# althonos/pyopal

Hardware: AMD Instinct MI355X
Metric: GCUPS (billion DP cells/s) SW score-only, 53aa query vs 1Mx300aa DB (higher is better)
Workload: dtype u16; 1 GPU; sw_score q53 (README.md:86) vs 1000000x300 uniform-random proteins per GPU, BLOSUM62, gap_open 3, gap_extend 1; value: blocking miopalSearch, scores in the caller's pinned host array (value_device_results: scores left in HBM); targets_per_gpu=1000000, target_length=300, query_length=53

## Files before the change

### pyopal_amd/csrc/common.h

```cpp
#pragma once
#include <hip/hip_runtime.h>
#include <stdint.h>
#include "launch_layer.h"

namespace miopal {

constexpr int kLanes = 64;
constexpr int kGroupTargets = 128;
constexpr int kMaxAlphabet = 32;
constexpr int kMaxStripRows = 64;

enum Region : int { kLastCell = 0, kLastRow = 1, kLastRowCol = 2, kAllCells = 3 };
struct DpRules {
    int topGap;
    int leftGap;
    int floor0;
    int region;
};

struct InterseqArgs {
    const uint2* pack;
    const int64_t* groupOff;
    const int* groupChunks;
    int nGroups;
// ... 17 lines not shown
    int* unitFlags;
    uint2* unitPartial;
    int scoreBias;
    int biasedLimit;
    int biasedZero;
    int capGroups, capChunks;
    int tailThrottle;
    unsigned long long* stripKeys;
    int* stripAbort;
    int stripAbortAt;
    int* stripGaveUp;
    int batchGroups;
    const int32_t* known;
    int32_t* directOut;
    int32_t* directEndI;
    int32_t* directEndJ;
    const int32_t* directIds;
    int directN;
    int splitMode;
    int splitBlocks;
    const int64_t* chunkPrefix;
    uint4* splitState;
    int* splitFlags;
    int stripSpinCap;
    int faultUnit1;
    unsigned long long* stripTiming;
    uint2* boundary[2];
    const int64_t* boundaryOff;
};

struct BatchArgs {
    const uint2* pack;
    const int64_t* groupOff;
    const int* groupChunks;
    const int32_t* lens;
    const int32_t* ids;
    int nPacked;
    int64_t sliceStart;
    const int16_t* profiles;
    int nSymbols;
    const int* qLens;
    const int* qRows;
    int nQueries;
    int unitsPerQuery;
    const int* unitFirst;
    int* unitCounter;
// ... 163 lines not shown
    kSwShifted = 6
};
constexpr int kSwShiftZero = 0x1000;
constexpr int kUnsignedDiagZero = 0x1000;
hipError_t launchInterseq(const InterseqArgs& a, int rowsPerStrip, int waves, InterseqFlavour flavour,
                          bool locate, hipStream_t stream);
__host__ __device__ constexpr int pairRowSlots(int rowsPerStrip) { return ((rowsPerStrip + 3) / 4) | 1; }
__host__ __device__ constexpr size_t pairLdsBytes(int rowsPerStrip, int nSymbols) {
    return (size_t)nSymbols * nSymbols * pairRowSlots(rowsPerStrip) * 16;
}
bool interseqPairFits(int rowsPerStrip, int nSymbols);
enum PairFlavour : int {
    kPairSwInt16 = 0,
    kPairSwHalf = 1,
    kPairSwBiased = 2,
    kPairGlobalBiased = 3,
    kPairSwStrips = 4,
    kPairGlobalStrips = 5
};
constexpr int kPairStripsFirst = 32;
constexpr int kPairStripsMaxRows = 52, kPairStripsMaxRowsLoc = 48;
constexpr int kPairStripsMaxRowsKnown = 40;
constexpr int kPairWavesPerGroup = 12;
inline size_t splitStateBytes(int rows) { return (size_t)((2 * rows + 1 + 3) / 4) * kLanes * 16; }
constexpr int kBiasedScoreLimit = 25600;
constexpr int kBiasedMaxMagnitude = 1024;
constexpr int kBiasedMaxExt = 512;
constexpr int kBiasedMaxStepUp = 0x1000;
constexpr int kBiasedPad = -1024;
constexpr int kLocZeroPattern = 0x0C00;
constexpr int kLocGuardBand = 0x0800;
constexpr int kLocMaxShift = 4096;
inline int locRowBitsHost(int rows) { return rows <= 16 ? 4 : rows <= 32 ? 5 : 6; }
hipError_t launchInterseqPair(const InterseqArgs& a, int rowsPerStrip, PairFlavour flavour, int computeUnits,
                              hipStream_t stream, bool locate = false);
struct ArithSwI16;
struct ArithSwF16;
struct ArithI16;
struct ArithI16Diag;
struct ArithU16Diag;
struct ArithSwU16;
constexpr int kPairUnitCounts = 8, kPairUnitSpan = 2 * kPairUnitCounts;
template <typename Arith, bool TRACK_ALL, bool LOC>
hipError_t launchFlavour(const InterseqArgs& a, int rowsPerStrip, int waves, hipStream_t stream);
template <typename Arith>
hipError_t launchPairFlavour(const InterseqArgs& a, int rowsPerStrip, int computeUnits, hipStream_t stream);
// ... 81 lines not shown
```

### pyopal_amd/csrc/host.hip

```cpp
#include <algorithm>
#include <atomic>
#include <chrono>
#include <condition_variable>
#if defined(__x86_64__)
#include <immintrin.h>
#endif
#include <cstdarg>
#include <cstdio>
#include <cstdlib>
#include <cstring>
#include <deque>
#include <functional>
#include <exception>
#include <ctime>
#include <list>
#include <map>
#include <memory>
#include <mutex>
#include <new>
#include <numeric>
#include <string>
#include <sys/mman.h>
#include <thread>
#include <vector>
// ... 527 lines not shown
    for (int k = 0; k < 4; ++k) counts[k] = g_lastRouting[k];
}

int miopalLastFullRouting(void) { return g_lastFullRouting; }

void miopalLastBatchRouting(int64_t counts[4]) {
    if (!counts) return;
    for (int k = 0; k < 4; ++k) counts[k] = g_lastBatchRouting[k];
}

int miopalLastKernelTime(MiopalDb* db, float* ms) {
    if (!db || !ms) return 0;
    std::lock_guard<std::mutex> g(db->timingMutex);
    *ms = 0.f;
    Workspace* ws = db->lastTimed;
    if (!ws) return 0;
    int n = 0;
    for (auto& ev : ws->timings) {
        float t = 0.f;
        if (hipEventSynchronize(ev.second) == hipSuccess &&
            hipEventElapsedTime(&t, ev.first, ev.second) == hipSuccess) {
            *ms += t;
            ++n;
        }
        (void)hipEventDestroy(ev.first);
        (void)hipEventDestroy(ev.second);
    }
    ws->timings.clear();
    return n;
}

int miopalSearchDeviceScores(MiopalDb* db, const unsigned char* query, int queryLength, int gapOpen,
                             int gapExt, const int* scoreMatrix, int alphabetLength, int mode,
                             int64_t start, int64_t end, int* deviceScores, void* stream) {
    return guarded([&]() -> int {
    RC_TRY(validate(db, query, queryLength, scoreMatrix, alphabetLength, OPAL_SEARCH_SCORE, mode, start, end));
    if (end == start) return 0;
    if (!deviceScores) return fail(MIOPAL_ERR_BAD_ARGUMENT, "null device score buffer");
    HIP_TRY(hipSetDevice(db->device));
    WorkspaceLease lease(db);
    RC_TRY(lease.acquireExternal((hipStream_t)stream));
    Search s{db, lease.ws, (hipStream_t)stream, query, queryLength, gapOpen, gapExt, alphabetLength,
             OPAL_SEARCH_SCORE, mode, scoreMatrix, start, end, end - start};
    RC_TRY(s.prepare());
    RC_TRY(s.scorePass((int32_t*)deviceScores, nullptr, nullptr));
    if (s.d_stripError) {
// ... 473 lines not shown
```

### pyopal_amd/csrc/host_search.inc

```
static inline int reservedCus(const MiopalDb* db) {
    const int opt = db->optReserveCus.load(std::memory_order_relaxed);
    if (opt >= 0) return opt;
    if (const char* r = tuned(Tune::RESERVE_CUS)) return std::max(0, atoi(r));
    return -1;
}
static inline bool smallSearchAllowed(const MiopalDb* db) {
    const int opt = db->optSmallSearch.load(std::memory_order_relaxed);
    if (opt >= 0) return opt != 0;
    return !tuned(Tune::NO_SMALL_SEARCH);
}

struct Search {
    MiopalDb* db;
    Workspace* ws;
    hipStream_t stream;
    const unsigned char* query;
    int Q, open, ext, A, searchType, mode;
    const int* matrix;
    int64_t start, end;
    int64_t n;
    const int* pssmRows = nullptr;
    int at(int i, int t) const { return pssmRows ? pssmRows[(size_t)i * A + t] : matrix[query[i] * A + t]; }
    int maxScore = 0, minScore = 0;
    int64_t balancedChunks = 0;
// ... 781 lines not shown
            ia.directN = view->nPacked;
            ia.overflow = nullptr;
            directScatter = true;
        }
        const PairFlavour pf = p.globalPair ? kPairGlobalBiased : p.biased ? kPairSwBiased : p.halfFloat ? kPairSwHalf : kPairSwInt16;
        size_t splitFlags = 0;
        if (pf == kPairSwBiased && !p.locate) {
            const char* cs = tuned(Tune::COLUMN_SPLIT);
            const bool recompute = cs && !strcmp(cs, "recompute");
            const int forced = cs && !recompute ? std::max(0, atoi(cs)) : 0;
            int64_t chunks = view->totalChunks;
            for (int g = 0; g < p.firstGroup; ++g) chunks -= view->groupChunksHost[g];
            const int blocks = (int)std::min<int64_t>(forced > 0 ? std::min(forced, pairUnits) : std::max(1, std::min(pairUnits, ia.nGroups)),
                                                      chunks / kPairWavesPerGroup);
            const int64_t wavefronts = (int64_t)blocks * kPairWavesPerGroup;
            if (blocks >= 1 && (recompute || forced > 0 || (!cs && uniform && chunks / wavefronts >= longest))) {
                void* st;
                RC_TRY(ws->get(kSplitState, (size_t)(wavefronts + 1) * splitStateBytes(p.pairRows), &st));
                ia.splitMode = recompute ? 2 : 1;
                ia.splitBlocks = blocks;
                ia.chunkPrefix = view->d_chunkPrefix;
                ia.splitState = (uint4*)st;
                splitFlags = (size_t)wavefronts + 1;
            }
        }
        RC_TRY(ws->get(kWorkCounter, (1 + splitFlags) * sizeof(int), &wc));
        HIP_TRY(hipMemsetAsync(wc, 0, (1 + splitFlags) * sizeof(int), stream));
        ia.workCounter = (int*)wc;
        if (splitFlags) ia.splitFlags = (int*)wc + 1;
        unsigned long long* simdFinish = nullptr;
        const int finishSlots = 1 + 4 * pairUnits;
        if (pf == kPairSwBiased && tuned(Tune::STRIP_TIMING)) {
            void* tb;
            RC_TRY(ws->get(kStripTiming, finishSlots * sizeof(unsigned long long), &tb));
            HIP_TRY(hipMemsetAsync(tb, 0, finishSlots * sizeof(unsigned long long), stream));
            HIP_TRY(hipMemsetAsync(tb, 0xff, sizeof(unsigned long long), stream));
            ia.stripTiming = simdFinish = (unsigned long long*)tb;
        }
        g_lastRouting[1] = 2 + (int)pf + (ia.splitMode ? 64 : 0);
        const hipError_t pe = tuned(Tune::TEST_REFUSE_PAIR_LAUNCH)
                                  ? hipErrorInvalidValue
                                  : launchInterseqPair(ia, (p.biased || p.globalPair) ? p.pairRows : p.rows, pf, pairUnits, stream, p.locate);
        if (pe == hipSuccess && simdFinish) {
            std::vector<unsigned long long> t((size_t)finishSlots);
            HIP_TRY(hipMemcpyAsync(t.data(), simdFinish, t.size() * sizeof(unsigned long long), hipMemcpyDeviceToHost, stream));
            HIP_TRY(hipStreamSynchronize(stream));
            double sum = 0, last = 0, first = 1e30;
            int n = 0;
            for (int i = 1; i < finishSlots; ++i) {
                if (t[i] == 0) continue;
                const double us = (double)(t[i] - t[0]) / 100.0;
                sum += us;
                last = std::max(last, us);
                first = std::min(first, us);
                ++n;
            }
            if (n > 0)
                fprintf(stderr, "[miopal] headline timing (%d SIMDs, %d groups, %d rows): finish mean %.1f us  first %.1f  last %.1f  "
                                "last - mean %.1f us\n",
                        n, ia.nGroups, p.pairRows, sum / n, first, last, last - sum / n);
        }
        done->directScatter = directScatter;
        done->launch = pe;
        return 0;
    }

    int scatterResults(const View* view, const ScorePlan& p, const InterseqArgs& ia, const PassBuffers& b, bool sideEmpty, bool forked,
                       bool directScatter, int32_t* d_score, int32_t* d_endI, int32_t* d_endJ) {
        const int nScatter = view->nPacked - p.packedSkip;
        if (p.keyed) {
            if (p.firstPos != 0 || !sideEmpty || forked)
                return fail(MIOPAL_ERR_INTERNAL, "segmented view with side jobs");
            HIP_TRY(launchScatterKeyed(ia.score, ia.endI, ia.endJ, (const uint8_t*)b.vo, view->d_ids,
                                       view->d_segStart, nScatter, start, (unsigned long long*)b.keys,
                                       p.mayOverflow ? (int32_t*)b.ct : nullptr, stream, p.keyBias));
            HIP_TRY(launchDecodeKeys((const unsigned long long*)b.keys, (int)n, d_score, d_endI, d_endJ, stream, p.keyBias));
        } else if (!directScatter) {
            HIP_TRY(launchScatter(ia.score + p.packedSkip, (const uint8_t*)b.vo + p.packedSkip, view->d_ids + p.packedSkip,
                                  nScatter, start, d_score, p.mayOverflow ? (int32_t*)b.ct : nullptr, p.overlap > 0,
                                  stream));
            if (p.locate)
                HIP_TRY(launchScatterEnds(ia.endI + p.packedSkip, ia.endJ + p.packedSkip, view->d_ids + p.packedSkip,
                                          nScatter, start, d_endI, d_endJ, stream));
// ... 33 lines not shown
        if (p.keyed) {
            RC_TRY(ws->get(kKeys, (size_t)n * sizeof(unsigned long long), &b.keys));
            HIP_TRY(hipMemsetAsync(b.keys, 0, (size_t)n * sizeof(unsigned long long), stream));
        } else if (p.overlap > 0) {
            if (p.keyBias) HIP_TRY(launchFillInt32(d_score, (int)n, INT32_MIN, stream));
            else HIP_TRY(hipMemsetAsync(d_score, 0, (size_t)n * sizeof(int32_t), stream));
        }
        planGeneralStrips(view.get(), p);
        planSwPairStrips(view.get(), useHalf, p);
        planGlobalPairStrips(view.get(), useHalf, p);
        planSideCut(view.get(), p, sideJobs);

        if (view->nGroups > p.firstGroup) {
            planLanes(view.get(), useHalf, p, jobs, sideJobs);
            const std::vector<int16_t> prof = buildProfile(p);
            bool forked = sideForked;
            bool directScatter = false;
            RC_TRY(forkSideJobs(p, sideJobs, d_score, d_endI, d_endJ, &forked, spt));
            InterseqArgs ia{};
            RC_TRY(prepareLaunch(view.get(), p, prof, b, ia));
            const bool timed = db->profiling.load() != 0;
            EventPair ev;
            if (timed) {
                HIP_TRY(hipEventCreate(&ev.e0));
                HIP_TRY(hipEventCreate(&ev.e1));
                HIP_TRY(hipEventRecord(ev.e0, stream));
            }
            g_lastRouting[1] = 1 + 32 * (int)p.flavour;
            if (p.pairStrips) {
                StripsLaunch sl;
                RC_TRY(prepareStripsLaunch(p, ia, &sl));
                hipError_t pe = hipSuccess;
                if (p.probeEnds) {
                    StripsProbe probe;
                    RC_TRY(probeStripsEnds(p, ia, sl, &probe));
                    pe = probe.launch;
                    if (pe == hipSuccess && 2 * probe.beyond >= probe.lanes) {
                        stripsEndsDeclined = true;
                        twoPassEnds = !tuned(Tune::NO_TWO_PASS_ENDS);
                        return scorePassImpl(d_score, d_endI, d_endJ, useHalf);
                    }
                }
                if (pe == hipSuccess) RC_TRY(launchStripsSweeps(view.get(), p, ia, sl, &pe));
                if (pe != hipSuccess) {
                    (void)hipGetLastError();
                    (p.globalStrips ? globalStripsRefused : pairStripsRefused) = true;
                    if (tuned(Tune::VERBOSE))
                        fprintf(stderr, "miopal: multi-strip pair-table kernel refused (%s), using the general kernel\n",
// ... 72 lines not shown
```

### pyopal_amd/csrc/host_types.inc

```
struct View {
    int64_t start = 0, end = 0;
    int overlap = 0;
    int stride = 0;
    int32_t* d_segStart = nullptr;
    int nPacked = 0;
    int nGroups = 0;
    int maxPackedLen = 0;
    std::vector<int> groupChunksHost;
    int64_t totalChunks = 0;
    std::vector<int32_t> ids;
    std::vector<int32_t> longIds;
    int32_t* d_ids = nullptr;
    int32_t* d_lens = nullptr;
    uint2* d_pack = nullptr;
    int64_t* d_groupOff = nullptr;
    int* d_groupChunks = nullptr;
    int64_t* d_boundaryOff = nullptr;
    int64_t* d_chunkPrefix = nullptr;
    size_t deviceBytes = 0;
    void* d_meta = nullptr;
    bool packPending = false;
    PackArgs pendingPack{};
    size_t packCap = 0, metaCap = 0;
    ~View() {
        if (d_pack) (void)hipFree(d_pack);
        if (d_meta) (void)hipFree(d_meta);
    }
};

}

struct MiopalDb {
    int device = 0;
    int ordinal = 0;
    std::atomic<int> optReserveCus{-1};
    std::atomic<int> optSmallSearch{-1};
    int alphabet = 0;
    int64_t count = 0;
    int64_t total = 0;
    int64_t maxLen = 0;
    int computeUnits = 256;
    std::vector<int64_t> offsets;
    uint8_t* d_residues = nullptr;
    int64_t* d_offsets = nullptr;
    size_t residueCap = 0, offsetsCap = 0;
    std::vector<std::pair<void*, size_t>> spareBlocks;

    struct ViewSlot {
        int64_t start, end;
// ... 133 lines not shown
```

### pyopal_amd/csrc/host_workspace.inc

```
enum Slot {
    kQuery, kMatrix, kProfile, kViewScore, kViewOvf, kCounter, kBoundary0, kBoundary1,
    kScore, kEndI, kEndJ, kJobs, kPairB0, kPairB1, kAuxJobs, kAuxPairB0, kAuxPairB1, kRScore, kRI, kRJ, kDirs, kOps, kOpsOff,
    kOpsLen, kOvfHost, kWorkCounter, kViewEndI, kViewEndJ, kStartQ, kStartT, kMismatch, kCompactOps, kTraceScore, kOpsTotals, kSortBins, kSortedJobs, kScanOrder, kKeys, kHeadWaves, kHeadDirs, kUnitState, kUnitPartial, kStripKeys,
    kPairStripState, kPairStripPartial, kPairStripSpare, kAuxPairStripState, kAuxPairStripPartial, kPairStripError, kStripTiming,
    kBatchProfiles, kBatchMeta, kBatchOverflow,
    kPairListQ, kPairListT, kPairListTOff, kPairListQBase, kPairListQOff, kPairListBoundary,
    kTopScratch,
    kPssmRows,
    kSplitState,
    kSlots
};

namespace unpack {
#if defined(__x86_64__)
__attribute__((target("bmi2"))) inline void pieces(uint8_t* dst, const uint8_t* packed, int64_t n8) {
    for (int64_t k = 0; k < n8; ++k) {
        uint16_t w;
        memcpy(&w, packed + 2 * k, 2);
        const uint64_t v = __builtin_ia32_pdep_di((uint64_t)w, 0x0303030303030303ull);
        memcpy(dst + 8 * k, &v, 8);
    }
}
inline bool havePdep() {
    static const bool yes = __builtin_cpu_supports("bmi2");
    return yes;
}
__attribute__((target("avx512f,avx512bw,avx512vbmi"))) inline void pieces64(uint8_t* dst, const uint8_t* packed, int64_t n64,
                                                                              bool stream) {
    const __m512i from = _mm512_set1_epi64((long long)0x0e0c0a0806040200ull);
    const __m512i low2 = _mm512_set1_epi8(3);
    if (stream) {
        for (int64_t k = 0; k < n64; ++k) {
// ... 202 lines not shown
inline bool haveAvx512() { return false; }
#endif
inline void copyLarge(void* dst, const void* src, size_t bytes) {
    if (bytes < (256u << 10) || !haveAvx512()) {
        memcpy(dst, src, bytes);
        return;
    }
    uint8_t* d = (uint8_t*)dst;
    const uint8_t* s = (const uint8_t*)src;
    const size_t lead = (64 - (reinterpret_cast<uintptr_t>(d) & 63)) & 63;
    memcpy(d, s, lead);
    const size_t lines = (bytes - lead) / 64;
    streamLines(d + lead, s + lead, lines);
    memcpy(d + lead + 64 * lines, s + lead + 64 * lines, bytes - lead - 64 * lines);
}
}

struct Workspace {
    hipStream_t stream = nullptr;
    bool ownsStream = false;
    void* buf[kSlots] = {};
    size_t cap[kSlots] = {};
    uint64_t usedBy[kSlots] = {};
    uint64_t leaseStamp = 0;
    std::mutex busy;
    std::vector<std::pair<hipEvent_t, hipEvent_t>> timings;
    hipStream_t aux = nullptr;
    hipEvent_t evFork = nullptr, evJoin = nullptr;

    void* pinned = nullptr;
    size_t pinnedCap = 0, pinnedUsed = 0;
    uint64_t stagingGeneration = 0;
    struct Pending { void* dst; size_t off, bytes; bool onAux = false; };
    std::vector<Pending> pending;
    std::vector<int32_t> hostScratchA, hostScratchB;

    static void copyOut(void* dst, const char* src, size_t bytes) {
        constexpr size_t kPiece = 4u << 20;
        if (bytes < 2 * kPiece) {
            unpack::copyLarge(dst, src, bytes);
            return;
        }
        const int nThreads = (int)std::min<size_t>(4, bytes / kPiece);
        const size_t share = ((bytes / nThreads) + 4095) & ~(size_t)4095;
        std::vector<std::thread> pool;
        for (int t = 1; t < nThreads; ++t) {
            const size_t lo = share * t, hi = std::min(bytes, lo + share);
            if (lo >= hi) continue;
            try {
// ... 120 lines not shown
            (void)hipGetLastError();
            least = greatest = 0;
        }
        if (greatest != least) HIP_TRY(hipStreamCreateWithPriority(&aux, hipStreamNonBlocking, greatest));
        else HIP_TRY(hipStreamCreateWithFlags(&aux, hipStreamNonBlocking));
        HIP_TRY(hipEventCreateWithFlags(&evFork, hipEventDisableTiming));
        HIP_TRY(hipEventCreateWithFlags(&evJoin, hipEventDisableTiming));
        return 0;
    }

    int get(int slot, size_t bytes, void** out) {
        if (bytes == 0) bytes = 16;
        usedBy[slot] = leaseStamp;
        if (cap[slot] < bytes) {
            if (buf[slot]) {
                HIP_TRY(hipStreamSynchronize(stream));
                HIP_TRY(hipFree(buf[slot]));
                buf[slot] = nullptr;
                cap[slot] = 0;
            }
            size_t want = bytes + bytes / 8 + 256;
            HIP_TRY(hipMalloc(&buf[slot], want));
            cap[slot] = want;
            if (want > (512u << 20) && tuned(Tune::VERBOSE))
                fprintf(stderr, "miopal: workspace slot %d grows to %zu MiB\n", slot, want >> 20);
        }
        *out = buf[slot];
        return 0;
    }
    bool tryGet(int slot, size_t bytes, void** out) {
        usedBy[slot] = leaseStamp;
        if (cap[slot] >= bytes) {
            *out = buf[slot];
            return true;
        }
        if (buf[slot]) {
            (void)hipStreamSynchronize(stream);
            (void)hipFree(buf[slot]);
            buf[slot] = nullptr;
            cap[slot] = 0;
        }
        if (hipMalloc(&buf[slot], bytes) != hipSuccess) {
            (void)hipGetLastError();
            buf[slot] = nullptr;
            return false;
        }
        cap[slot] = bytes;
        if (bytes > (512u << 20) && tuned(Tune::VERBOSE))
            fprintf(stderr, "miopal: workspace slot %d grows to %zu MiB\n", slot, bytes >> 20);
        *out = buf[slot];
        return true;
    }
    size_t bytes() const {
        size_t t = 0;
        for (size_t c : cap) t += c;
        return t;
    }
    size_t trimTo(size_t keep, bool staleOnly = false) {
        size_t freed = 0;
        for (int pass = 0; pass < (staleOnly ? 1 : 2); ++pass)
        while (bytes() > keep) {
            int big = -1;
            for (int k = 0; k < kSlots; ++k)
                if (buf[k] && (pass == 1 || usedBy[k] != leaseStamp) && (big < 0 || cap[k] > cap[big])) big = k;
            if (big < 0) break;
            (void)hipFree(buf[big]);
            freed += cap[big];
            buf[big] = nullptr;
            cap[big] = 0;
        }
        return freed;
    }
    ~Workspace() {
        for (auto& ev : timings) {
            (void)hipEventDestroy(ev.first);
            (void)hipEventDestroy(ev.second);
        }
        for (void* p : buf)
            if (p) (void)hipFree(p);
        if (pinned) (void)hipHostFree(pinned);
        if (evFork) (void)hipEventDestroy(evFork);
        if (evJoin) (void)hipEventDestroy(evJoin);
        if (aux) (void)hipStreamDestroy(aux);
        if (ownsStream && stream) (void)hipStreamDestroy(stream);
    }
};
```

### pyopal_amd/csrc/interseq_impl.h

```cpp
#pragma once
#include <algorithm>

#include <type_traits>

#include "common.h"

namespace miopal {

typedef short s16x2 __attribute__((ext_vector_type(2)));
typedef unsigned short u16x2 __attribute__((ext_vector_type(2)));
typedef _Float16 f16x2 __attribute__((ext_vector_type(2)));

static __device__ __forceinline__ uint32_t pk_add_sat_i16(uint32_t a, uint32_t b) {
    s16x2 r = __builtin_elementwise_add_sat(__builtin_bit_cast(s16x2, a), __builtin_bit_cast(s16x2, b));
    return __builtin_bit_cast(uint32_t, r);
}
static __device__ __forceinline__ uint32_t pk_sub_sat_i16(uint32_t a, uint32_t b) {
    s16x2 r = __builtin_elementwise_sub_sat(__builtin_bit_cast(s16x2, a), __builtin_bit_cast(s16x2, b));
    return __builtin_bit_cast(uint32_t, r);
}
static __device__ __forceinline__ uint32_t pk_max_i16(uint32_t a, uint32_t b) {
    s16x2 r = __builtin_elementwise_max(__builtin_bit_cast(s16x2, a), __builtin_bit_cast(s16x2, b));
    return __builtin_bit_cast(uint32_t, r);
}
// ... 905 lines not shown
    __device__ __forceinline__ void begin(int lane) const {
        if (MIOPAL_STRIP_PACE && lane == 0) *mine = 0;
    }
    __device__ __forceinline__ void end(int lane) const {
        if (MIOPAL_STRIP_PACE && lane == 0) *mine = INT32_MAX;
    }
    __device__ __forceinline__ void step(int c, int lane, bool fixed) const {
        if (!MIOPAL_STRIP_PACE || fixed) return;
        if (lane == 0) *mine = c;
        const int4 p = *simdRow;
        const int behind = __builtin_amdgcn_readfirstlane(min(min(p.x, p.y), min(p.z, p.w)));
        if (c <= behind) __builtin_amdgcn_s_setprio(2);
        else __builtin_amdgcn_s_setprio(0);
    }
};

#ifndef MIOPAL_HEADLINE_PACE
#define MIOPAL_HEADLINE_PACE 1
#endif
#ifndef MIOPAL_HEADLINE_TIMING
#define MIOPAL_HEADLINE_TIMING 0
#endif

struct SplitState {
    __amdgpu_buffer_rsrc_t rsrc;
    __device__ __forceinline__ explicit SplitState(void* base)
        : rsrc(__builtin_amdgcn_make_buffer_rsrc(base, 0, 0x7ffffff0, 0x00020000)) {}
    static __device__ __forceinline__ int at(int quad) {
        int offset = quad * (kLanes * 16);
        asm volatile("" : "+s"(offset));
        return offset;
    }
    __device__ __forceinline__ StripU4 load(int quad, int lane) const {
        return __builtin_amdgcn_raw_buffer_load_b128(rsrc, lane * 16, at(quad), 16 );
    }
    __device__ __forceinline__ void store(int quad, int lane, StripU4 v) const {
        __builtin_amdgcn_raw_buffer_store_b128(v, rsrc, lane * 16, at(quad), 16 );
    }
};
constexpr int kSplitPolls = 256;
__host__ __device__ constexpr int splitStateQuads(int rows) { return (2 * rows + 1 + 3) / 4; }

template <int R, bool LOC, bool SPLIT = false>
__global__ __launch_bounds__(kPairWaves * kLanes) void interseq_pair_biased_kernel(InterseqArgs a) {
    static_assert(!(SPLIT && LOC), "the column split carries no end locations");
    constexpr int SLOTS = PairLayout<R>::kRowSlots;
    constexpr int NB4 = (R + 3) / 4;
    constexpr int kBits = LOC ? locRowBits(R) : 0;
    constexpr int kRowMask = (1 << kBits) - 1;
    extern __shared__ uint4 pairs[];
#if MIOPAL_HEADLINE_TIMING
    const unsigned long long born = __builtin_amdgcn_s_memrealtime();
#endif

    const int lane = threadIdx.x & 63;
    const int nSym = a.nSymbols;
    const int ext = a.gapExt << kBits;
    const uint32_t ext2 = both(ext), openMinusExt2 = both((a.gapOpen << kBits) - ext);
    const uint32_t zero2 = both(LOC ? kLocZero : kBiasedZero);

    {
        const int16_t* gp = a.profile;
        uint32_t* pw = reinterpret_cast<uint32_t*>(pairs);
        const int total = nSym * nSym * R;
        for (int idx = threadIdx.x; idx < total; idx += kPairWaves * kLanes) {
            const int row = idx / R, r = idx - row * R;
            const int tA = row / nSym, tB = row - tA * nSym;
            constexpr int kPadPattern = LOC ? -kLocGuard : kBiasedPadScore;
            const int vA = gp[tA * a.qPad + r], vB = gp[tB * a.qPad + r];
            const int sA = (vA == kBiasedPadScore ? kPadPattern : vA << kBits) + ext;
            const int sB = (vB == kBiasedPadScore ? kPadPattern : vB << kBits) + ext;
            pw[row * (SLOTS * 4) + r] = (uint32_t)(sB * 65536 + sA);
        }
    }
    int* simdTaken = reinterpret_cast<int*>(pairs + nSym * nSym * SLOTS);
    if (threadIdx.x < 4) simdTaken[threadIdx.x] = 0;
    __syncthreads();
    SimdPace pace;
    if (MIOPAL_HEADLINE_PACE) pace.init(simdTaken + 4, lane);

    const int wave = __builtin_amdgcn_readfirstlane((int)(threadIdx.x >> 6));
    constexpr int kTier[4][3] = {{0, 6, 11}, {1, 7, 8}, {2, 5, 9}, {3, 4, 10}};
    const int tier = kTier[wave & 3][wave >> 2];
    const int firstDynamic = kPairWaves * gridDim.x;
    const int simd = (int)__builtin_amdgcn_s_getreg(4 | (4 << 6) | ((2 - 1) << 11)) & 3;
    bool firstRound = true;
    int splitW = 0, gLo = 0, gHi = 0, cutLo = 0, cutHi = 0, gWhole = 0, phase = 0, paceAfter = 0;
    if constexpr (SPLIT) {
        const int64_t* pre = a.chunkPrefix + a.groupBase;
        const uint32_t C = (uint32_t)(pre[a.nGroups] - pre[0]);
        const uint32_t W = kPairWaves * gridDim.x, each = C / W, rest = C % W;
        splitW = kPairWaves * (int)blockIdx.x + wave;
        const uint32_t lo = splitW * each + splitW * rest / W, hi = (splitW + 1) * each + (splitW + 1) * rest / W;
        const float groupsPerChunk = (float)a.nGroups / (float)(C > 0 ? C : 1);
        auto groupOf = [&](uint32_t x) {
            int k = (int)((float)x * groupsPerChunk);
            k = k < 0 ? 0 : k > a.nGroups ? a.nGroups : k;
            while (k > 0 && (uint32_t)(pre[k] - pre[0]) > x) --k;
            while (k < a.nGroups && (uint32_t)(pre[k + 1] - pre[0]) <= x) ++k;
            return k;
        };
        gLo = __builtin_amdgcn_readfirstlane(groupOf(lo));
        gHi = __builtin_amdgcn_readfirstlane(groupOf(hi));
        cutLo = __builtin_amdgcn_readfirstlane((int)(lo - (uint32_t)(pre[gLo] - pre[0])));
        cutHi = __builtin_amdgcn_readfirstlane((int)(hi - (uint32_t)(pre[gHi] - pre[0])));
        gWhole = cutLo > 0 ? gLo + 1 : gLo;
        paceAfter = __builtin_amdgcn_readfirstlane((int)(hi - lo));
        if (lo == hi) phase = 3;
    }
    for (;;) {
        int g;
        int cBegin = 0, cEnd = 0;
        bool consume = false, produce = false;
        if constexpr (SPLIT) {
            if (phase == 0) {
// ... 42 lines not shown
                if (a.tailThrottle > 0) take = atomicAdd(&simdTaken[simd], 1) < a.tailThrottle;
                g = take ? atomicAdd(a.workCounter, 1) : INT32_MAX - firstDynamic;
            }
            g = __builtin_amdgcn_readfirstlane(g) + firstDynamic;
            if (g >= a.nGroups) break;
            g += a.groupBase;
        }
        const uint2* pack = a.pack + a.groupOff[g];
        const int nChunks = a.groupChunks[g];
        if (nChunks > a.priorityChunks) __builtin_amdgcn_s_setprio(3);
        else __builtin_amdgcn_s_setprio(0);
        uint32_t best = 0u;
        int colA = -1, colB = -1;
        uint32_t fl = zero2 - ext2;
        int shift = -ext;
        uint32_t H[R], E[R];
        if constexpr (SPLIT) {
            if (cEnd == 0) cEnd = nChunks;
            paceAfter -= cEnd - cBegin;
            if (consume) {
                bool there = false;
                if (a.splitMode != 2) {
                    for (int poll = 0; poll < kSplitPolls && !there; ++poll) {
                        there = stripPoll(a.splitFlags + splitW) != 0;
                        if (!there) __builtin_amdgcn_s_sleep(16);
                    }
                }
                if (!there) {
                    consume = false;
                    cBegin = 0;
                }
            }
        }
        if (SPLIT && consume) {
            fl = zero2;
            shift = 0;
            const SplitState mine(a.splitState + (size_t)splitW * splitStateQuads(R) * kLanes);
#pragma unroll
            for (int q = 0; q < splitStateQuads(R); ++q) {
                if (q % 7 == 0 && q > 0) asm volatile("s_waitcnt vmcnt(0)" ::: "memory");
                const StripU4 v = mine.load(q, lane);
#pragma unroll
                for (int k = 0; k < 4; ++k) {
                    const int i = 4 * q + k;
                    const uint32_t x = k == 0 ? v.x : k == 1 ? v.y : k == 2 ? v.z : v.w;
                    if (i < R) H[i] = x;
                    else if (i < 2 * R) E[i - R] = x;
// ... 9 lines not shown
        }
        const int cFirst = SPLIT ? cBegin : 0, cLast = SPLIT ? cEnd : nChunks;
        uint2 cur = pack[(size_t)cFirst * kLanes + lane];
        auto rowOf = [&](uint32_t tA, uint32_t tB) -> const uint4* {
            const uint32_t rowIdx = __umul24(tA, (uint32_t)nSym) + tB;
            return reinterpret_cast<const uint4*>(reinterpret_cast<const char*>(pairs) +
                                                  __umul24(rowIdx, (uint32_t)(SLOTS * 16)));
        };
#ifndef MIOPAL_PAIR_AHEAD
#define MIOPAL_PAIR_AHEAD 3
#endif
#ifndef MIOPAL_PAIR_XCOL
#define MIOPAL_PAIR_XCOL 1
#endif
        constexpr int kWant = LOC ? (R > 62 ? 1 : R > 58 ? 2 : MIOPAL_PAIR_AHEAD) : (R > 60 ? 2 : MIOPAL_PAIR_AHEAD);
        constexpr int kAhead = NB4 > kWant ? kWant : 1;
        constexpr bool kAcross = MIOPAL_PAIR_XCOL != 0;
        const uint4* prowNext = rowOf(cur.x & 0xffu, cur.y & 0xffu);
        uint4 vn[kAhead];
        if (kAcross) {
#pragma unroll
            for (int k = 0; k < kAhead; ++k) vn[k] = prowNext[k];
        }
        for (int c = cFirst; c < cLast; ++c) {
            uint2 nxt = {0, 0};
            if (c + 1 < nChunks) nxt = pack[(size_t)(c + 1) * kLanes + lane];
            if (MIOPAL_HEADLINE_PACE) pace.step(c - cLast - (SPLIT ? paceAfter : 0), lane, nChunks > a.priorityChunks);
            uint32_t ra = cur.x, rb = cur.y;
#pragma unroll 1
            for (int cc = 0; cc < 4; ++cc) {
                const uint4* prow = prowNext;
                uint4 v[NB4];
#pragma unroll
                for (int k = 0; k < kAhead; ++k) v[k] = kAcross ? vn[k] : prow[k];
                ra = cc < 3 ? ra >> 8 : nxt.x;
                rb = cc < 3 ? rb >> 8 : nxt.y;
                prowNext = rowOf(ra & 0xffu, rb & 0xffu);
                auto score = [&](int r) -> uint32_t {
                    const uint4 x = v[r >> 2];
                    const int k = r & 3;
                    return k == 0 ? x.x : k == 1 ? x.y : k == 2 ? x.z : x.w;
                };
                uint32_t dsum = fl + score(0);
                fl += ext2;
                uint32_t fl1 = fl + ext2;
                asm volatile("" : "+v"(fl1));
// ... 46 lines not shown
                const uint32_t d = both(shift);
#pragma unroll
                for (int r = 0; r < R; ++r) {
                    H[r] -= d;
                    E[r] -= d;
                }
                fl -= d;
                shift = 0;
            }
        }
        if constexpr (SPLIT) {
            if (produce) {
                const uint32_t d = both(shift);
                const SplitState next(a.splitState + (size_t)(splitW + 1) * splitStateQuads(R) * kLanes);
#pragma unroll
                for (int q = 0; q < splitStateQuads(R); ++q) {
                    auto word = [&](int i) -> uint32_t {
                        if (i < R) return H[i] - d;
                        if (i < 2 * R) return E[i - R] - d;
                        return i == 2 * R ? best : 0u;
                    };
                    next.store(q, lane, StripU4{word(4 * q), word(4 * q + 1), word(4 * q + 2), word(4 * q + 3)});
                }
                stripPublish(a.splitFlags + splitW + 1, 1, lane);
                continue;
            }
        }
        const int lo = (int)(best & 0xffffu) >> kBits, hi = (int)(best >> 16) >> kBits;
        const size_t base = (size_t)g * kGroupTargets;
        if (a.directOut) {
            const int posA = (int)base + lane, posB = posA + kLanes;
            if (posA < a.directN) {
                const int id = a.directIds[posA];
                a.directOut[id] = lo;
                if constexpr (LOC) {
                    a.directEndI[id] = colA < 0 ? -1 : kRowMask - (int)(best & kRowMask);
                    a.directEndJ[id] = colA;
                }
            }
            if (posB < a.directN) {
                const int id = a.directIds[posB];
                a.directOut[id] = hi;
                if constexpr (LOC) {
                    a.directEndI[id] = colB < 0 ? -1 : kRowMask - (int)((best >> 16) & kRowMask);
                    a.directEndJ[id] = colB;
                }
            }
            continue;
        }
        a.score[base + lane] = lo;
        a.score[base + kLanes + lane] = hi;
        if constexpr (LOC) {
            a.endI[base + lane] = colA < 0 ? -1 : kRowMask - (int)(best & kRowMask);
            a.endI[base + kLanes + lane] = colB < 0 ? -1 : kRowMask - (int)((best >> 16) & kRowMask);
            a.endJ[base + lane] = colA;
            a.endJ[base + kLanes + lane] = colB;
        }
        if (a.overflow) {
            a.overflow[base + lane] = lo >= a.biasedLimit;
            a.overflow[base + kLanes + lane] = hi >= a.biasedLimit;
        }
    }
    if (MIOPAL_HEADLINE_PACE && lane == 0) *pace.mine = INT32_MAX;
#if MIOPAL_HEADLINE_TIMING
    if (a.stripTiming && lane == 0) {
        atomicMin(a.stripTiming, born);
        atomicMax(a.stripTiming + 1 + blockIdx.x * 4 + simd, (unsigned long long)__builtin_amdgcn_s_memrealtime());
    }
#endif
}

template <int R, bool LOC>
static hipError_t launchPairBiasedR(const InterseqArgs& a, int computeUnits, hipStream_t stream) {
    const size_t lds = PairLayout<R>::bytes(a.nSymbols) + 16 + kPaceInts * sizeof(int);
    if (const hipError_t e = allowFullLds<&interseq_pair_biased_kernel<R, LOC>>(); e != hipSuccess) return e;
    const int blocks = std::max(1, std::min(computeUnits, a.nGroups));
    hipLaunchKernelGGL((interseq_pair_biased_kernel<R, LOC>), dim3(blocks), dim3(kPairWaves * kLanes), lds, stream, a);
    return hipGetLastError();
}

template <int R>
static hipError_t launchPairBiasedSplitR(const InterseqArgs& a, hipStream_t stream) {
    const size_t lds = PairLayout<R>::bytes(a.nSymbols) + 16 + kPaceInts * sizeof(int);
    if (const hipError_t e = allowFullLds<&interseq_pair_biased_kernel<R, false, true>>(); e != hipSuccess) return e;
    if (a.splitBlocks < 1 || !a.chunkPrefix || !a.splitState || !a.splitFlags) return hipErrorInvalidValue;
    hipLaunchKernelGGL((interseq_pair_biased_kernel<R, false, true>), dim3(a.splitBlocks), dim3(kPairWaves * kLanes), lds, stream, a);
    return hipGetLastError();
}

template <int kLo, bool LOC>
hipError_t launchPairBiased(const InterseqArgs& a, int rowsPerStrip, int computeUnits, hipStream_t stream) {
    if (a.nStrips != 1) return hipErrorInvalidValue;
    if constexpr (!LOC) {
        if (a.splitMode != 0)
            return dispatchRows<kLo, 2, kPairUnitCounts>(rowsPerStrip, [&](auto r) { return launchPairBiasedSplitR<r>(a, stream); });
    }
    return dispatchRows<kLo, 2, kPairUnitCounts>(rowsPerStrip, [&](auto r) { return launchPairBiasedR<r, LOC>(a, computeUnits, stream); });
}

#ifndef MIOPAL_STRIP_ROWS_AHEAD
#define MIOPAL_STRIP_ROWS_AHEAD 2
#endif
#ifndef MIOPAL_STRIP_SLEEP
#define MIOPAL_STRIP_SLEEP 8
#endif
#ifndef MIOPAL_STRIP_SLACK
#define MIOPAL_STRIP_SLACK 0
#endif
// ... 954 lines not shown
```

### pyopal_amd/csrc/tuning.h

```cpp
#pragma once
#include <atomic>

namespace miopal {

#define MIOPAL_TUNING_SWITCHES(X)                                                                          \
    X(COLUMN_SPLIT) X(DEVICE) X(FORCE_LANE_PER_PAIR) X(HOST_THREADS) X(HOST_TRACEBACK) X(NO_ASYNC_SHARES) X(NO_BIASED)     \
    X(NO_CALLER_PINNED) X(NO_DIAG_SHIFT) X(NO_DIRECT_SCATTER) X(NO_EARLY_HOST_SHARE) X(NO_GLOBAL_STRIPS)   \
    X(NO_HOST_SCATTER) X(NO_HUGEPAGE) X(NO_HYBRID_TRACE) X(NO_JOBS_AHEAD) X(NO_ONE_LAUNCH)                 \
    X(NO_PACKED_HW_SCAN) X(NO_PACKED_SCAN) X(NO_PACKED_TRACE) X(NO_PAIR_STRIPS) X(NO_PAIR_STRIP_UNITS)     \
    X(NO_PAIR_TABLE) X(NO_PERPAIR) X(NO_PERPAIR_PROFILE) X(NO_SCAN_ORDER) X(NO_SCAN_REFILL)                \
    X(NO_SEGMENTS) X(NO_SIDE_COPIES) X(NO_SIDE_STREAM) X(NO_SMALL_SEARCH) X(NO_SORT_BY_ROWS)               \
    X(NO_SW_SHIFT) X(NO_TWO_PASS_ENDS) X(NO_UNPACK_CREW) X(NO_VIEW_PREFETCH) X(ONE_LAUNCH_GROUP)           \
    X(PAIR_STRIPS) X(PARKED_WORKSPACE_MB) X(PHASE_TIMING) X(RESERVE_CUS) X(SEARCH_UNDER_UPLOAD)            \
    X(SPARE_HANDLE_MB) X(STRIPS) X(STRIP_TIMING) X(TAIL_THROTTLE) X(TEST_REFUSE_PAIR_LAUNCH)               \
    X(TWO_PASS_ENDS) X(UNITS) X(UPLOAD_PIECE_KB) X(UPLOAD_STREAMS) X(UPLOAD_THREADS) X(VERBOSE)            \
    X(VIEW_CACHE_MB)

enum class Tune : int {
#define X(name) name,
    MIOPAL_TUNING_SWITCHES(X)
#undef X
    kCount
};

const char* tuned(Tune key);

}
```

Baseline: 11010 GCUPS.

## Precompute split plans, reuse split flags by generation, speed pair-table build

```diff
diff --git a/pyopal_amd/csrc/common.h b/pyopal_amd/csrc/common.h
--- a/pyopal_amd/csrc/common.h
+++ b/pyopal_amd/csrc/common.h
@@ -63,6 +63,8 @@
     const int64_t* chunkPrefix;
     uint4* splitState;
     int* splitFlags;
+    const int* splitPlan;
+    int splitGeneration;
     int stripSpinCap;
     int faultUnit1;
     unsigned long long* stripTiming;
@@ -272,6 +274,8 @@
 constexpr int kPairStripsMaxRows = 52, kPairStripsMaxRowsLoc = 48;
 constexpr int kPairStripsMaxRowsKnown = 40;
 constexpr int kPairWavesPerGroup = 12;
+constexpr int kHeadlinePhaseSlots = 6;
+constexpr int kSplitPlanInts = 8;
 inline size_t splitStateBytes(int rows) { return (size_t)((2 * rows + 1 + 3) / 4) * kLanes * 16; }
 constexpr int kBiasedScoreLimit = 25600;
 constexpr int kBiasedMaxMagnitude = 1024;
diff --git a/pyopal_amd/csrc/host.hip b/pyopal_amd/csrc/host.hip
--- a/pyopal_amd/csrc/host.hip
+++ b/pyopal_amd/csrc/host.hip
@@ -573,6 +573,8 @@
             hipEventElapsedTime(&t, ev.first, ev.second) == hipSuccess) {
             *ms += t;
             ++n;
+            ws->spareEvents.push_back(ev);
+            continue;
         }
         (void)hipEventDestroy(ev.first);
         (void)hipEventDestroy(ev.second);
diff --git a/pyopal_amd/csrc/host_search.inc b/pyopal_amd/csrc/host_search.inc
--- a/pyopal_amd/csrc/host_search.inc
+++ b/pyopal_amd/csrc/host_search.inc
@@ -827,14 +827,15 @@
                 ia.chunkPrefix = view->d_chunkPrefix;
                 ia.splitState = (uint4*)st;
                 splitFlags = (size_t)wavefronts + 1;
-            }
-        }
-        RC_TRY(ws->get(kWorkCounter, (1 + splitFlags) * sizeof(int), &wc));
-        HIP_TRY(hipMemsetAsync(wc, 0, (1 + splitFlags) * sizeof(int), stream));
+                if (!tuned(Tune::NO_SPLIT_PLAN)) RC_TRY(view->splitPlanFor(p.firstGroup, (int)wavefronts, &ia.splitPlan));
+            }
+        }
+        RC_TRY(ws->get(kWorkCounter, sizeof(int), &wc));
         ia.workCounter = (int*)wc;
-        if (splitFlags) ia.splitFlags = (int*)wc + 1;
+        if (splitFlags) RC_TRY(ws->splitFlagsFor(splitFlags, stream, &ia.splitFlags, &ia.splitGeneration));
+        else HIP_TRY(hipMemsetAsync(wc, 0, sizeof(int), stream));
         unsigned long long* simdFinish = nullptr;
-        const int finishSlots = 1 + 4 * pairUnits;
+        const int finishSlots = 1 + kHeadlinePhaseSlots + 4 * pairUnits;
         if (pf == kPairSwBiased && tuned(Tune::STRIP_TIMING)) {
             void* tb;
             RC_TRY(ws->get(kStripTiming, finishSlots * sizeof(unsigned long long), &tb));
@@ -852,7 +853,7 @@
             HIP_TRY(hipStreamSynchronize(stream));
             double sum = 0, last = 0, first = 1e30;
             int n = 0;
-            for (int i = 1; i < finishSlots; ++i) {
+            for (int i = 1 + kHeadlinePhaseSlots; i < finishSlots; ++i) {
                 if (t[i] == 0) continue;
                 const double us = (double)(t[i] - t[0]) / 100.0;
                 sum += us;
@@ -864,6 +865,11 @@
                 fprintf(stderr, "[miopal] headline timing (%d SIMDs, %d groups, %d rows): finish mean %.1f us  first %.1f  last %.1f  "
                                 "last - mean %.1f us\n",
                         n, ia.nGroups, p.pairRows, sum / n, first, last, last - sum / n);
+            if (t[3] > 0)
+                fprintf(stderr, "[miopal] headline phases (%llu wavefronts, %llu with a piece): start -> table done max %.2f us  mean %.2f  "
+                                "table done -> first column max %.2f us  mean %.2f\n",
+                        t[3], t[6], (double)t[1] / 100.0, (double)t[2] / 100.0 / (double)t[3], (double)t[4] / 100.0,
+                        t[6] ? (double)t[5] / 100.0 / (double)t[6] : 0.0);
         }
         done->directScatter = directScatter;
         done->launch = pe;
@@ -943,8 +949,18 @@
             const bool timed = db->profiling.load() != 0;
             EventPair ev;
             if (timed) {
-                HIP_TRY(hipEventCreate(&ev.e0));
-                HIP_TRY(hipEventCreate(&ev.e1));
+                {
+                    std::lock_guard<std::mutex> g(db->timingMutex);
+                    if (!ws->spareEvents.empty()) {
+                        ev.e0 = ws->spareEvents.back().first;
+                        ev.e1 = ws->spareEvents.back().second;
+                        ws->spareEvents.pop_back();
+                    }
+                }
+                if (!ev.e0) {
+                    HIP_TRY(hipEventCreate(&ev.e0));
+                    HIP_TRY(hipEventCreate(&ev.e1));
+                }
                 HIP_TRY(hipEventRecord(ev.e0, stream));
             }
             g_lastRouting[1] = 1 + 32 * (int)p.flavour;
diff --git a/pyopal_amd/csrc/host_types.inc b/pyopal_amd/csrc/host_types.inc
--- a/pyopal_amd/csrc/host_types.inc
+++ b/pyopal_amd/csrc/host_types.inc
@@ -22,9 +22,47 @@
     bool packPending = false;
     PackArgs pendingPack{};
     size_t packCap = 0, metaCap = 0;
+    mutable std::mutex planMutex;
+    mutable std::map<std::pair<int, int>, int*> splitPlans;
+    int splitPlanFor(int firstGroup, int wavefronts, const int** d_plan) const {
+        std::lock_guard<std::mutex> g(planMutex);
+        auto it = splitPlans.find({firstGroup, wavefronts});
+        if (it == splitPlans.end()) {
+            const std::vector<int> plan = splitPlanHost(firstGroup, wavefronts);
+            int* d = nullptr;
+            HIP_TRY(hipMalloc(&d, plan.size() * sizeof(int)));
+            if (const hipError_t e = hipMemcpy(d, plan.data(), plan.size() * sizeof(int), hipMemcpyHostToDevice); e != hipSuccess) {
+                (void)hipFree(d);
+                HIP_TRY(e);
+            }
+            it = splitPlans.emplace(std::make_pair(firstGroup, wavefronts), d).first;
+        }
+        *d_plan = it->second;
+        return 0;
+    }
+    std::vector<int> splitPlanHost(int firstGroup, int wavefronts) const {
+        const int groups = nGroups - firstGroup;
+        std::vector<uint32_t> pre((size_t)groups + 1, 0u);
+        for (int k = 0; k < groups; ++k) pre[(size_t)k + 1] = pre[(size_t)k] + (uint32_t)groupChunksHost[(size_t)(firstGroup + k)];
+        const uint32_t C = pre[(size_t)groups], W = (uint32_t)wavefronts, each = C / W, rest = C % W;
+        auto groupOf = [&](uint32_t x) { return (int)(std::upper_bound(pre.begin(), pre.end(), x) - pre.begin()) - 1; };
+        std::vector<int> plan((size_t)wavefronts * kSplitPlanInts, 0);
+        for (uint32_t w = 0; w < W; ++w) {
+            const uint32_t lo = w * each + w * rest / W, hi = (w + 1) * each + (w + 1) * rest / W;
+            const int gLo = groupOf(lo), gHi = groupOf(hi);
+            int* e = &plan[(size_t)w * kSplitPlanInts];
+            e[0] = gLo;
+            e[1] = (int)(lo - pre[(size_t)gLo]);
+            e[2] = gHi;
+            e[3] = (int)(hi - pre[(size_t)gHi]);
+            e[4] = (int)(hi - lo);
+        }
+        return plan;
+    }
     ~View() {
         if (d_pack) (void)hipFree(d_pack);
         if (d_meta) (void)hipFree(d_meta);
+        for (auto& entry : splitPlans) (void)hipFree(entry.second);
     }
 };
 
diff --git a/pyopal_amd/csrc/host_workspace.inc b/pyopal_amd/csrc/host_workspace.inc
--- a/pyopal_amd/csrc/host_workspace.inc
+++ b/pyopal_amd/csrc/host_workspace.inc
@@ -8,6 +8,7 @@
     kTopScratch,
     kPssmRows,
     kSplitState,
+    kSplitFlags,
     kSlots
 };
 
@@ -256,9 +257,11 @@
     void* buf[kSlots] = {};
     size_t cap[kSlots] = {};
     uint64_t usedBy[kSlots] = {};
+    uint64_t allocCount[kSlots] = {};
     uint64_t leaseStamp = 0;
     std::mutex busy;
     std::vector<std::pair<hipEvent_t, hipEvent_t>> timings;
+    std::vector<std::pair<hipEvent_t, hipEvent_t>> spareEvents;
     hipStream_t aux = nullptr;
     hipEvent_t evFork = nullptr, evJoin = nullptr;
 
@@ -425,10 +428,36 @@
             size_t want = bytes + bytes / 8 + 256;
             HIP_TRY(hipMalloc(&buf[slot], want));
             cap[slot] = want;
+            ++allocCount[slot];
             if (want > (512u << 20) && tuned(Tune::VERBOSE))
                 fprintf(stderr, "miopal: workspace slot %d grows to %zu MiB\n", slot, want >> 20);
         }
         *out = buf[slot];
+        return 0;
+    }
+    int splitGeneration = 0;
+    uint64_t splitFlagsAlloc = 0;
+    const char* splitPresetSeen = nullptr;
+    int splitFlagsFor(size_t ints, hipStream_t on, int** flags, int* generation) {
+        void* f;
+        RC_TRY(get(kSplitFlags, ints * sizeof(int), &f));
+        bool zero = splitFlagsAlloc != allocCount[kSplitFlags] || splitGeneration == INT32_MAX;
+        int next = zero ? 1 : splitGeneration + 1;
+        if (const char* preset = tuned(Tune::TEST_SPLIT_GENERATION); preset != splitPresetSeen) {
+            splitPresetSeen = preset;
+            const long long n = preset ? atoll(preset) : 0;
+            if (n >= 1 && n <= INT32_MAX) {
+                next = (int)n;
+                zero = true;
+            }
+        }
+        if (zero) {
+            HIP_TRY(hipMemsetAsync(f, 0, cap[kSplitFlags], on));
+            splitFlagsAlloc = allocCount[kSplitFlags];
+        }
+        splitGeneration = next;
+        *flags = (int*)f;
+        *generation = next;
         return 0;
     }
     bool tryGet(int slot, size_t bytes, void** out) {
@@ -449,6 +478,7 @@
             return false;
         }
         cap[slot] = bytes;
+        ++allocCount[slot];
         if (bytes > (512u << 20) && tuned(Tune::VERBOSE))
             fprintf(stderr, "miopal: workspace slot %d grows to %zu MiB\n", slot, bytes >> 20);
         *out = buf[slot];
@@ -475,10 +505,11 @@
         return freed;
     }
     ~Workspace() {
-        for (auto& ev : timings) {
-            (void)hipEventDestroy(ev.first);
-            (void)hipEventDestroy(ev.second);
-        }
+        for (auto* list : {&timings, &spareEvents})
+            for (auto& ev : *list) {
+                (void)hipEventDestroy(ev.first);
+                (void)hipEventDestroy(ev.second);
+            }
         for (void* p : buf)
             if (p) (void)hipFree(p);
         if (pinned) (void)hipHostFree(pinned);
diff --git a/pyopal_amd/csrc/interseq_impl.h b/pyopal_amd/csrc/interseq_impl.h
--- a/pyopal_amd/csrc/interseq_impl.h
+++ b/pyopal_amd/csrc/interseq_impl.h
@@ -951,6 +951,47 @@
 #define MIOPAL_HEADLINE_TIMING 0
 #endif
 
+constexpr int kTableHeld = 32;
+template <int R, int SLOTS, int kBits, bool LOC>
+static __device__ __forceinline__ void buildBiasedPairTable(uint32_t* pw, const int16_t* gp, int nSym, int qPad, int ext,
+                                                            int lane, int wave) {
+    constexpr int kPadPattern = LOC ? -kLocGuard : kBiasedPadScore;
+    auto pattern = [&](int v) { return (v == kBiasedPadScore ? kPadPattern : v << kBits) + ext; };
+    if (lane >= R) lane = R - 1;
+    const int last = nSym - 1;
+    const uint32_t entryStep = (uint32_t)qPad * 2u;
+    const uint32_t rowStep = (uint32_t)nSym * (SLOTS * 16);
+    auto entry = [&](uint32_t at) -> int { return *reinterpret_cast<const int16_t*>(reinterpret_cast<const char*>(gp) + at); };
+    for (int tA0 = 0; tA0 < nSym; tA0 += kTableHeld) {
+        int sA[kTableHeld];
+        uint32_t at = (uint32_t)(tA0 * qPad + lane) * 2u;
+#pragma unroll
+        for (int k = 0; k < kTableHeld; ++k) {
+            sA[k] = entry(at);
+            at += tA0 + k < last ? entryStep : 0u;
+            asm volatile("" : "+v"(at));
+        }
+        int vB = entry((uint32_t)((wave < last ? wave : last) * qPad + lane) * 2u);
+#pragma unroll
+        for (int k = 0; k < kTableHeld; ++k) sA[k] = pattern(sA[k]);
+        for (int tB = wave; tB < nSym; tB += kPairWaves) {
+            const int ahead = tB + kPairWaves;
+            const int vBnext = entry((uint32_t)((ahead < last ? ahead : last) * qPad + lane) * 2u);
+            const int sB = pattern(vB) * 65536;
+            uint32_t to = (uint32_t)((tA0 * nSym + tB) * (SLOTS * 4) + lane) * 4u;
+            int held = nSym - tA0;
+            asm volatile("" : "+s"(held));
+#pragma unroll
+            for (int k = 0; k < kTableHeld; ++k) {
+                if (k < held) *reinterpret_cast<uint32_t*>(reinterpret_cast<char*>(pw) + to) = (uint32_t)(sB + sA[k]);
+                to += rowStep;
+                asm volatile("" : "+v"(to));
+            }
+            vB = vBnext;
+        }
+    }
+}
+
 struct SplitState {
     __amdgpu_buffer_rsrc_t rsrc;
     __device__ __forceinline__ explicit SplitState(void* base)
@@ -988,38 +1029,63 @@
     const uint32_t ext2 = both(ext), openMinusExt2 = both((a.gapOpen << kBits) - ext);
     const uint32_t zero2 = both(LOC ? kLocZero : kBiasedZero);
 
-    {
-        const int16_t* gp = a.profile;
-        uint32_t* pw = reinterpret_cast<uint32_t*>(pairs);
-        const int total = nSym * nSym * R;
-        for (int idx = threadIdx.x; idx < total; idx += kPairWaves * kLanes) {
-            const int row = idx / R, r = idx - row * R;
-            const int tA = row / nSym, tB = row - tA * nSym;
-            constexpr int kPadPattern = LOC ? -kLocGuard : kBiasedPadScore;
-            const int vA = gp[tA * a.qPad + r], vB = gp[tB * a.qPad + r];
-            const int sA = (vA == kBiasedPadScore ? kPadPattern : vA << kBits) + ext;
-            const int sB = (vB == kBiasedPadScore ? kPadPattern : vB << kBits) + ext;
-            pw[row * (SLOTS * 4) + r] = (uint32_t)(sB * 65536 + sA);
-        }
-    }
+    const int wave = __builtin_amdgcn_readfirstlane((int)(threadIdx.x >> 6));
+    int splitW = 0;
+    [[maybe_unused]] int planned[kSplitPlanInts] = {};
+    [[maybe_unused]] int plannedChunks = 0;
+    [[maybe_unused]] uint2 plannedCur = {0, 0};
+    if constexpr (SPLIT) {
+        splitW = kPairWaves * (int)blockIdx.x + wave;
+        if (a.splitPlan) {
+            const int* entry = a.splitPlan + (size_t)splitW * kSplitPlanInts;
+#pragma unroll
+            for (int k = 0; k < kSplitPlanInts; ++k) planned[k] = __builtin_amdgcn_readfirstlane(entry[k]);
+            const int pLo = planned[0], pCutLo = planned[1], pHi = planned[2], pCutHi = planned[3];
+            const int pWhole = pCutLo > 0 ? pLo + 1 : pLo;
+            int plannedG = -1, plannedC = 0;
+            if (planned[4] > 0) {
+                if (pLo == pHi) plannedG = pLo, plannedC = pCutLo;
+                else if (pCutHi > 0) plannedG = pHi;
+                else if (pWhole < pHi) plannedG = pWhole;
+                else if (pCutLo > 0) plannedG = pLo, plannedC = pCutLo;
+            }
+            if (plannedG >= 0) {
+                plannedG += a.groupBase;
+                plannedChunks = a.groupChunks[plannedG];
+                plannedCur = (a.pack + a.groupOff[plannedG])[(size_t)plannedC * kLanes + lane];
+            }
+        }
+    }
+    buildBiasedPairTable<R, SLOTS, kBits, LOC>(reinterpret_cast<uint32_t*>(pairs), a.profile, nSym, a.qPad, ext, lane, wave);
     int* simdTaken = reinterpret_cast<int*>(pairs + nSym * nSym * SLOTS);
     if (threadIdx.x < 4) simdTaken[threadIdx.x] = 0;
     __syncthreads();
+#if MIOPAL_HEADLINE_TIMING
+    const unsigned long long tableDone = __builtin_amdgcn_s_memrealtime();
+    unsigned long long firstColumn = 0;
+#endif
     SimdPace pace;
     if (MIOPAL_HEADLINE_PACE) pace.init(simdTaken + 4, lane);
 
-    const int wave = __builtin_amdgcn_readfirstlane((int)(threadIdx.x >> 6));
     constexpr int kTier[4][3] = {{0, 6, 11}, {1, 7, 8}, {2, 5, 9}, {3, 4, 10}};
     const int tier = kTier[wave & 3][wave >> 2];
     const int firstDynamic = kPairWaves * gridDim.x;
     const int simd = (int)__builtin_amdgcn_s_getreg(4 | (4 << 6) | ((2 - 1) << 11)) & 3;
     bool firstRound = true;
-    int splitW = 0, gLo = 0, gHi = 0, cutLo = 0, cutHi = 0, gWhole = 0, phase = 0, paceAfter = 0;
-    if constexpr (SPLIT) {
+    int gLo = 0, gHi = 0, cutLo = 0, cutHi = 0, gWhole = 0, phase = 0, paceAfter = 0;
+    if (SPLIT && a.splitPlan) {
+        gLo = planned[0];
+        cutLo = planned[1];
+        gHi = planned[2];
+        cutHi = planned[3];
+        gWhole = cutLo > 0 ? gLo + 1 : gLo;
+        paceAfter = planned[4];
+        if (paceAfter == 0) phase = 3;
+        asm volatile("" ::"s"(plannedChunks), "v"(plannedCur.x), "v"(plannedCur.y));
+    } else if constexpr (SPLIT) {
         const int64_t* pre = a.chunkPrefix + a.groupBase;
         const uint32_t C = (uint32_t)(pre[a.nGroups] - pre[0]);
         const uint32_t W = kPairWaves * gridDim.x, each = C / W, rest = C % W;
-        splitW = kPairWaves * (int)blockIdx.x + wave;
         const uint32_t lo = splitW * each + splitW * rest / W, hi = (splitW + 1) * each + (splitW + 1) * rest / W;
         const float groupsPerChunk = (float)a.nGroups / (float)(C > 0 ? C : 1);
         auto groupOf = [&](uint32_t x) {
@@ -1108,7 +1174,7 @@
                 bool there = false;
                 if (a.splitMode != 2) {
                     for (int poll = 0; poll < kSplitPolls && !there; ++poll) {
-                        there = stripPoll(a.splitFlags + splitW) != 0;
+                        there = stripPoll(a.splitFlags + splitW) == a.splitGeneration;
                         if (!there) __builtin_amdgcn_s_sleep(16);
                     }
                 }
@@ -1164,6 +1230,9 @@
 #pragma unroll
             for (int k = 0; k < kAhead; ++k) vn[k] = prowNext[k];
         }
+#if MIOPAL_HEADLINE_TIMING
+        if (firstColumn == 0) firstColumn = __builtin_amdgcn_s_memrealtime();
+#endif
         for (int c = cFirst; c < cLast; ++c) {
             uint2 nxt = {0, 0};
             if (c + 1 < nChunks) nxt = pack[(size_t)(c + 1) * kLanes + lane];
@@ -1256,7 +1325,7 @@
                     };
                     next.store(q, lane, StripU4{word(4 * q), word(4 * q + 1), word(4 * q + 2), word(4 * q + 3)});
                 }
-                stripPublish(a.splitFlags + splitW + 1, 1, lane);
+                stripPublish(a.splitFlags + splitW + 1, a.splitGeneration, lane);
                 continue;
             }
         }
@@ -1299,7 +1368,15 @@
 #if MIOPAL_HEADLINE_TIMING
     if (a.stripTiming && lane == 0) {
         atomicMin(a.stripTiming, born);
-        atomicMax(a.stripTiming + 1 + blockIdx.x * 4 + simd, (unsigned long long)__builtin_amdgcn_s_memrealtime());
+        atomicMax(a.stripTiming + 1, tableDone - born);
+        atomicAdd(a.stripTiming + 2, tableDone - born);
+        atomicAdd(a.stripTiming + 3, 1ull);
+        if (firstColumn != 0) {
+            atomicMax(a.stripTiming + 4, firstColumn - tableDone);
+            atomicAdd(a.stripTiming + 5, firstColumn - tableDone);
+            atomicAdd(a.stripTiming + 6, 1ull);
+        }
+        atomicMax(a.stripTiming + 1 + kHeadlinePhaseSlots + blockIdx.x * 4 + simd, (unsigned long long)__builtin_amdgcn_s_memrealtime());
     }
 #endif
 }
@@ -1317,7 +1394,7 @@
 static hipError_t launchPairBiasedSplitR(const InterseqArgs& a, hipStream_t stream) {
     const size_t lds = PairLayout<R>::bytes(a.nSymbols) + 16 + kPaceInts * sizeof(int);
     if (const hipError_t e = allowFullLds<&interseq_pair_biased_kernel<R, false, true>>(); e != hipSuccess) return e;
-    if (a.splitBlocks < 1 || !a.chunkPrefix || !a.splitState || !a.splitFlags) return hipErrorInvalidValue;
+    if (a.splitBlocks < 1 || !a.chunkPrefix || !a.splitState || !a.splitFlags || a.splitGeneration < 1) return hipErrorInvalidValue;
     hipLaunchKernelGGL((interseq_pair_biased_kernel<R, false, true>), dim3(a.splitBlocks), dim3(kPairWaves * kLanes), lds, stream, a);
     return hipGetLastError();
 }
diff --git a/pyopal_amd/csrc/tuning.h b/pyopal_amd/csrc/tuning.h
--- a/pyopal_amd/csrc/tuning.h
+++ b/pyopal_amd/csrc/tuning.h
@@ -10,9 +10,11 @@
     X(NO_PACKED_HW_SCAN) X(NO_PACKED_SCAN) X(NO_PACKED_TRACE) X(NO_PAIR_STRIPS) X(NO_PAIR_STRIP_UNITS)     \
     X(NO_PAIR_TABLE) X(NO_PERPAIR) X(NO_PERPAIR_PROFILE) X(NO_SCAN_ORDER) X(NO_SCAN_REFILL)                \
     X(NO_SEGMENTS) X(NO_SIDE_COPIES) X(NO_SIDE_STREAM) X(NO_SMALL_SEARCH) X(NO_SORT_BY_ROWS)               \
+    X(NO_SPLIT_PLAN)                                                                                       \
     X(NO_SW_SHIFT) X(NO_TWO_PASS_ENDS) X(NO_UNPACK_CREW) X(NO_VIEW_PREFETCH) X(ONE_LAUNCH_GROUP)           \
     X(PAIR_STRIPS) X(PARKED_WORKSPACE_MB) X(PHASE_TIMING) X(RESERVE_CUS) X(SEARCH_UNDER_UPLOAD)            \
     X(SPARE_HANDLE_MB) X(STRIPS) X(STRIP_TIMING) X(TAIL_THROTTLE) X(TEST_REFUSE_PAIR_LAUNCH)               \
+    X(TEST_SPLIT_GENERATION)                                                                               \
     X(TWO_PASS_ENDS) X(UNITS) X(UPLOAD_PIECE_KB) X(UPLOAD_STREAMS) X(UPLOAD_THREADS) X(VERBOSE)            \
     X(VIEW_CACHE_MB)
 
```

After: 11090 GCUPS, median of 6. Within noise of the previous version (+0.8%).
